# skyhehe123/SA-SSD

Hardware: NVIDIA H100
Metric: KITTI frames/sec (~20k pts, car_cfg voxel grid) (higher is better)
Workload: dtype f32

## Files before the change

### include/sassd_b200.h

```cpp
#ifndef SASSD_B200_H
#define SASSD_B200_H

#include <stddef.h>
#include <stdint.h>

#ifdef __cplusplus
extern "C" {
#endif

typedef void* sassd_stream_t;

enum {
    SASSD_OK = 0,
    SASSD_ERR_ARG = -1,
    SASSD_ERR_LAUNCH = -2,
    SASSD_ERR_WORKSPACE = -3,
    SASSD_ERR_UNSUPPORTED = -4
};

enum {
    SASSD_FLAG_VOXEL_CAP = 1,
    SASSD_FLAG_ROWS_CAP = 2,
    SASSD_FLAG_GUIDED_CAP = 4,
    SASSD_FLAG_NMS_CAP = 8,
// ... 77 lines not shown
                const float* shift, const int32_t* nbr, const int32_t* d_rows, float* out, sassd_stream_t stream);

size_t sassd_gconv_pack_bytes(int taps, int cin, int cout, int precision);
int sassd_gconv_pack(const float* weight, int taps, int cin, int cout, int precision, void* packed,
                     sassd_stream_t stream);

size_t sassd_conv2d_pack_bytes(int taps, int cin, int cout);
int sassd_conv2d_pack(const float* weight, int taps, int cin, int cout, void* packed, sassd_stream_t stream);
typedef struct {
    int32_t batch, H, W;
    int32_t cin, cin_stored;
    int32_t cout, taps, relu;
    int32_t out_f32_stride, out_split_ch;
    int32_t tile_order;
    int32_t n_split;
} sassd_conv2d_desc;
int sassd_conv2d_f16x3(const sassd_conv2d_desc* host_desc, const void* in_split, const void* wpack, const float* scale,
                       const float* shift, float* out_f32, void* out_split, sassd_stream_t stream);
#define SASSD_CONV2D_TILE_H 8
#define SASSD_CONV2D_TILE_W 16
#define SASSD_TILE_DIST_MAX 9
int sassd_conv2d_f16x3_occ(const sassd_conv2d_desc* host_desc, const void* in_split, const void* wpack,
                           const float* scale, const float* shift, float* out_f32, void* out_split,
                           const int32_t* tile_dist, int reach, const float* const_out, int32_t* counters,
                           sassd_stream_t stream);
int sassd_conv2d_f16x3_occ_bg(const sassd_conv2d_desc* host_desc, const void* in_split, const void* wpack,
                              const float* scale, const float* shift, float* out_f32, void* out_split,
                              const int32_t* tile_dist, int reach, const float* const_out, const void* bg_split,
                              const float* bg_f32, int32_t* counters, sassd_stream_t stream);
int sassd_sparse_to_bev_split(const float* feat, const int32_t* coors, const int32_t* d_rows, int rows_cap, int C,
// ... 166 lines not shown
```

### sa-ssd_b200/csrc/conv2d_tma.cu

```cuda
#include <cuda.h>

#include <cstdlib>

#include "tc_common.cuh"

namespace tma {

using namespace tc;

constexpr int TILE_H = SASSD_CONV2D_TILE_H, TILE_W = SASSD_CONV2D_TILE_W;
constexpr int BKC = 64;
constexpr int kConstTile = 1 << 30;
constexpr int kBgTile = 1 << 29;
constexpr int CONS_WARPS = CONS_THREADS / 32;
constexpr int W_LOAD = CONS_WARPS;

constexpr int A_ROWS = TILE_H + 2;
constexpr int A_PLANE_BYTES = A_ROWS * TILE_W * 128;
constexpr int A_STAGE_BYTES = 2 * A_PLANE_BYTES;

constexpr int FRAG_BLOCK_BYTES = 128 * 32;
constexpr int OUT_PITCH = 64 + 4;

template <int BN>
// ... 21 lines not shown
}

struct Conv2dArgs {
    const void* wpack;
    const float* scale;
    const float* shift;
    float* out_f32;
    __half* out_split;
    int batch, H, W, cin, cout, taps, relu, out_f32_stride, out_split_ch;
    const int* tile_dist;
    const float* cvec;
    int reach;
    int* counters;
    int tile_order;
    int nsplit;
};

struct Background {
    const __half* split;
    const float* f32;
};

__device__ __forceinline__ int tile_skip_flag(const Conv2dArgs& p, const Background& bg, int dist, int ty, int tx,
                                              int tiles_y, int tiles_x) {
    if (dist <= p.reach) return 0;
    if (p.reach < 2 || !(ty == 0 || ty == tiles_y - 1 || tx == 0 || tx == tiles_x - 1)) return kConstTile;
    return (bg.split || bg.f32) ? kBgTile : 0;
}

__device__ __forceinline__ void copy_background_unit(const Conv2dArgs& p, const Background& bg, int b, int ty, int tx,
// ... 56 lines not shown
                                                int nthreads) {
    if (!p.out_split || c0 >= p.out_split_ch) return;
    const int vpp = (p.out_split_ch - c0) >> 3;
    const size_t plane = (size_t)p.batch * p.H * p.W * p.out_split_ch;
    const uint4 zero = make_uint4(0u, 0u, 0u, 0u);
    for (int i = tid; i < TILE_H * TILE_W * vpp; i += nthreads) {
        const int pix = i / vpp;
        const int y = ty * TILE_H + pix / TILE_W, x = tx * TILE_W + pix % TILE_W;
        if (y >= p.H || x >= p.W) continue;
        __half* dst = p.out_split + (((size_t)b * p.H + y) * p.W + x) * p.out_split_ch + c0 + 8 * (i % vpp);
        *(uint4*)dst = zero;
        *(uint4*)(dst + plane) = zero;
    }
}

__device__ __forceinline__ void mma_chunk_x3_rs(float (&big)[64], float (&small)[64], const uint32_t (&w)[32],
                                                uint32_t x_hi, uint32_t x_lo) {
    const uint64_t dxh = make_desc(x_hi), dxl = make_desc(x_lo);
#pragma unroll
    for (int k = 0; k < 4; ++k) {
        const uint64_t ko = 2ull * (uint64_t)k;
        const uint32_t wh[4] = {w[8 * k], w[8 * k + 1], w[8 * k + 2], w[8 * k + 3]};
        const uint32_t wl[4] = {w[8 * k + 4], w[8 * k + 5], w[8 * k + 6], w[8 * k + 7]};
        wgmma_rs_n128(small, wh, dxl + ko);
        wgmma_rs_n128(small, wl, dxh + ko);
        wgmma_rs_n128(big, wh, dxh + ko);
    }
}

template <int BN>
__global__ void __launch_bounds__(Cfg2<BN>::THREADS, 1)
conv2d_tma_kernel(const __grid_constant__ CUtensorMap amap, const Conv2dArgs p, const Background bg) {
    using C = Cfg2<BN>;
    constexpr int A_STAGES = C::A_STAGES;
    extern __shared__ uint8_t smem_raw[];
    __shared__ int s_ncomp;
    __shared__ int s_walk[6];
    const uint32_t base = (smem_u32(smem_raw) + 1023u) & ~1023u;
    uint8_t* base_ptr = smem_raw + (base - smem_u32(smem_raw));
    const uint32_t b_ring = base + A_STAGES * A_STAGE_BYTES;
    const uint32_t bar_base = base + C::RING_BYTES;
    auto a_full = [&](int s) { return bar_base + 8u * s; };
    auto a_empty = [&](int s) { return bar_base + 8u * (A_STAGES + s); };
    auto b_full = [&](int s) { return bar_base + 8u * (2 * A_STAGES + s); };
    auto b_empty = [&](int s) { return bar_base + 8u * (2 * A_STAGES + C::B_STAGES + s); };

    pdl_launch_dependents();
    const int warp = __shfl_sync(0xffffffffu, (int)(threadIdx.x >> 5), 0), lane = threadIdx.x & 31;
    const int tiles_x = (p.W + TILE_W - 1) / TILE_W, tiles_y = (p.H + TILE_H - 1) / TILE_H;
    const int ntiles = p.batch * tiles_y * tiles_x;
    const int nsplit = p.nsplit, nunits = ntiles * nsplit;
    const int kchunks = (p.cin + BKC - 1) / BKC;
    const int nchunks = p.taps * kchunks;
    const int ncols = p.taps == 9 ? 3 : 1, nrows = ncols, halo = ncols / 2;

    if (threadIdx.x == 0) {
        for (int s = 0; s < A_STAGES; ++s) { mbar_init(a_full(s), 1); mbar_init(a_empty(s), 2); }
        for (int s = 0; s < C::B_STAGES; ++s) { mbar_init(b_full(s), 1); mbar_init(b_empty(s), 2); }
        fence_barrier_init();
        asm volatile("prefetch.tensormap [%0];" ::"l"(&amap) : "memory");
        s_walk[0] = s_walk[1] = nunits;
        s_walk[2] = s_walk[4] = nunits + blockIdx.x;
        s_walk[3] = 1;
        s_walk[5] = blockIdx.x;
    }
    __syncthreads();
    pdl_wait();

    uint32_t* verdict = (uint32_t*)(base_ptr + C::RING_BYTES + 256);
    uint16_t* order = (uint16_t*)(verdict + 2 * (C::ORDER_CAP / 32));
    const bool small_map = p.tile_dist != nullptr && ntiles <= C::ORDER_CAP;
    const bool use_order = p.tile_order && small_map;
    if (small_map) {
        const int nslots = (ntiles + 31) / 32;
#pragma unroll 1
        for (int i0 = 4 * warp; i0 < nslots; i0 += 4 * (C::THREADS / 32)) {
            int dist[4];
#pragma unroll
            for (int e = 0; e < 4; ++e) {
// ... 25 lines not shown
                    for (int i = 0; i < nslots; ++i) {
                        const int t = i * 32 + lane;
                        const uint32_t cst = verdict[i], bgm = verdict[C::ORDER_CAP / 32 + i];
                        const bool skip = ((cst | bgm) >> lane) & 1u;
                        const bool take = t < ntiles && (skip == (pass == 1));
                        const uint32_t m = __ballot_sync(0xffffffffu, take);
                        if (take) order[n + __popc(m & ((1u << lane) - 1u))] = word(t, cst, bgm);
                        n += __popc(m);
                    }
                    if (pass == 0 && lane == 0) s_ncomp = n;
                }
                if (lane == 0) {
                    constexpr int kTailAbsorb = 8;
                    const int G = gridDim.x, c = blockIdx.x;
                    const int ucomp = s_ncomp * nsplit;
                    const int heavy = ucomp % G, light = G - heavy;
                    const int absorb = heavy ? min(nunits - ucomp, kTailAbsorb * light) : 0;
                    const int s2 = ucomp + c - heavy, s3 = ucomp + absorb + c;
                    const int first_tail = (c >= heavy && s2 < ucomp + absorb) ? s2 : s3;
                    s_walk[0] = ucomp;
                    s_walk[1] = ucomp + absorb;
                    s_walk[2] = first_tail;
                    s_walk[3] = light;
                    s_walk[4] = s3;
                    s_walk[5] = c < ucomp ? c : first_tail;
                }
            } else {
#pragma unroll 1
                for (int i = 0; i < nslots; ++i) {
                    const int t = i * 32 + lane;
                    if (t < ntiles) order[t] = word(t, verdict[i], verdict[C::ORDER_CAP / 32 + i]);
                }
            }
        }
        __syncthreads();
    }
    auto next_unit = [&](int k) -> int {
        if (k < s_walk[0]) { k += gridDim.x; return k < s_walk[0] ? k : s_walk[2]; }
        if (k < s_walk[1]) { k += s_walk[3]; return k < s_walk[1] ? k : s_walk[4]; }
        return k + gridDim.x;
    };
    auto tile_ref = [&](int k) -> int {
        if (small_map) { const int v = order[k]; return (v & 0x3fff) | ((v & 0xc000) << 15); }
        if (!p.tile_dist) return k;
        return k | tile_skip_flag(p, bg, __ldg(&p.tile_dist[k]), (k / tiles_x) % tiles_y, k % tiles_x, tiles_y, tiles_x);
    };

    if (warp >= W_LOAD) {
        if constexpr (C::RS) {
            setmaxnreg_dec<40>();
            if (warp == W_LOAD + 1 && lane == 0) {
                constexpr uint32_t kStep = 2 * FRAG_BLOCK_BYTES;
                int b_stage = 0;
                uint32_t b_phase = 0;
                for (int k = s_walk[5]; k < nunits; k = next_unit(k)) {
                    if (tile_ref(k / nsplit) & (kConstTile | kBgTile)) continue;
                    const uint8_t* src = (const uint8_t*)p.wpack + (size_t)(k % nsplit) * kStep;
                    for (int q = 0; q < nchunks; ++q) {
                        mbar_wait(b_empty(b_stage), b_phase ^ 1u);
                        mbar_expect_tx(b_full(b_stage), C::B_STAGE_BYTES);
                        const uint32_t dst = b_ring + b_stage * C::B_STAGE_BYTES;
#pragma unroll 1
                        for (int s = 0; s < 4; ++s, src += (size_t)nsplit * kStep)
                            bulk_g2s(dst + s * kStep, src, kStep, b_full(b_stage));
                        if (++b_stage == C::B_STAGES) { b_stage = 0; b_phase ^= 1u; }
                    }
                }
            }
            if (warp != W_LOAD) return;
        }
        if (lane == 0) {
            int a_stage = 0, b_stage = 0;
            uint32_t a_phase = 0, b_phase = 0;
            const uint32_t a_bytes = 2u * (TILE_H + 2 * halo) * TILE_W * 128;
            for (int k = s_walk[5]; k < nunits; k = next_unit(k)) {
                const int ref = tile_ref(k / nsplit), half = k % nsplit;
                if (ref & (kConstTile | kBgTile)) continue;
                const int tile = ref;
                const int b = tile / (tiles_y * tiles_x);
                const int ty = (tile / tiles_x) % tiles_y, tx = tile % tiles_x;
                const int y0 = ty * TILE_H, x0 = tx * TILE_W;
                for (int col = 0; col < ncols; ++col) {
                    const int dx = col - halo;
                    for (int kc = 0; kc < kchunks; ++kc) {
                        mbar_wait(a_empty(a_stage), a_phase ^ 1u);
                        const uint32_t a_hi = base + a_stage * A_STAGE_BYTES;
                        mbar_expect_tx(a_full(a_stage), a_bytes);
                        tma_load_4d(a_hi, &amap, kc * BKC, x0 + dx, y0 - halo, b, a_full(a_stage));
                        tma_load_4d(a_hi + A_PLANE_BYTES, &amap, kc * BKC, x0 + dx, y0 - halo, p.batch + b, a_full(a_stage));
                        if (++a_stage == A_STAGES) { a_stage = 0; a_phase ^= 1u; }
// ... 10 lines not shown
#pragma unroll 1
                                for (int part = 0; part < 2; ++part)
#pragma unroll 1
                                    for (uint32_t o = 0; o < (uint32_t)C::B_TILE_BYTES; o += kPiece)
                                        bulk_g2s(b_dst + part * C::B_TILE_BYTES + o,
                                                 src + (size_t)part * nsplit * C::B_TILE_BYTES + o, kPiece, b_full(b_stage));
                                if (++b_stage == C::B_STAGES) { b_stage = 0; b_phase ^= 1u; }
                            }
                        }
                    }
                }
            }
        }
        if (p.out_split && nsplit * BN < p.out_split_ch) {
            __syncwarp();
            for (int k = s_walk[5]; k < nunits; k = next_unit(k)) {
                if (k % nsplit != nsplit - 1) continue;
                const int tile = tile_ref(k / nsplit) & ~(kConstTile | kBgTile);
                zero_split_tail(p, tile / (tiles_y * tiles_x), (tile / tiles_x) % tiles_y, tile % tiles_x, nsplit * BN,
                                lane, 32);
            }
        }
    } else {
        if constexpr (C::RS) setmaxnreg_inc<232>();
        const int wg = threadIdx.x >> 7, t = threadIdx.x & 127;
        const int rl0 = wg * 64 + (t >> 5) * 16 + ((t & 31) >> 2);
        const size_t plane = (size_t)p.batch * p.H * p.W * p.out_split_ch;
        float big[BN / 2], small[BN / 2];
        int a_stage = 0, b_stage = 0;
        uint32_t a_phase = 0, b_phase = 0;
        int computed = 0;
        for (int k = s_walk[5]; k < nunits; k = next_unit(k)) {
            const int ref = tile_ref(k / nsplit), n_off = (k % nsplit) * BN;
            const int tile = ref & ~(kConstTile | kBgTile);
            const bool const_tile = (ref & kConstTile) != 0;
            const int b = tile / (tiles_y * tiles_x);
            const int ty = (tile / tiles_x) % tiles_y, tx = tile % tiles_x;
            if (ref & kBgTile) continue;
            if (const_tile) {
                const int ncols = min(BN, p.out_split_ch - n_off);
                if (p.out_split && !p.out_f32 && (ncols == 64 || ncols == 128 || ncols == 256)) {
                    store_constant_unit<CONS_WARPS>(p, b, ty, tx, n_off, ncols, warp, lane);
                    continue;
                }
            } else {
                if (k % nsplit == 0) ++computed;
#pragma unroll
                for (int i = 0; i < BN / 2; ++i) { big[i] = 0.f; small[i] = 0.f; }
                int prev_b = -1, prev_a = -1, row = 0;
                if constexpr (C::RS) {
                    auto load_w = [&](uint32_t (&w)[32]) {
                        mbar_wait(b_full(b_stage), b_phase);
                        const uint32_t sw = (t & 4) * 4u;
                        const uint32_t src = b_ring + b_stage * C::B_STAGE_BYTES + wg * FRAG_BLOCK_BYTES + t * 32;
#pragma unroll
                        for (int s = 0; s < 4; ++s) {
                            const uint4 x = lds_v4(src + s * 2 * FRAG_BLOCK_BYTES + sw);
                            const uint4 y = lds_v4(src + s * 2 * FRAG_BLOCK_BYTES + (sw ^ 16u));
                            const uint4 h = sw ? y : x, l = sw ? x : y;
                            w[8 * s] = h.x; w[8 * s + 1] = h.y; w[8 * s + 2] = h.z; w[8 * s + 3] = h.w;
                            w[8 * s + 4] = l.x; w[8 * s + 5] = l.y; w[8 * s + 6] = l.z; w[8 * s + 7] = l.w;
                        }
                        named_bar_sync(3 + wg, 128);
                        if (t == 0) mbar_arrive(b_empty(b_stage));
                        if (++b_stage == C::B_STAGES) { b_stage = 0; b_phase ^= 1u; }
                    };
                    auto chunk = [&](uint32_t (&w)[32], uint32_t (&w_next)[32], int ch) {
                        if (row == 0) mbar_wait(a_full(a_stage), a_phase);
                        const uint32_t xh = base + a_stage * A_STAGE_BYTES + (uint32_t)row * (TILE_W * 128u);
                        wgmma_fence();
                        mma_chunk_x3_rs(big, small, w, xh, xh + A_PLANE_BYTES);
                        wgmma_commit();
                        wgmma_wait<1>();
                        fence_regs<32>(w_next);
                        if (t == 0 && prev_a >= 0) mbar_arrive(a_empty(prev_a));
                        if (ch + 1 < nchunks) load_w(w_next);
                        prev_a = -1;
                        if (++row == nrows) {
                            row = 0;
                            prev_a = a_stage;
                            if (++a_stage == A_STAGES) { a_stage = 0; a_phase ^= 1u; }
                        }
                    };
                    uint32_t wa[32], wb[32];
                    load_w(wa);
                    for (int ch = 0; ch < nchunks; ch += 2) {
                        chunk(wa, wb, ch);
// ... 24 lines not shown
                            row = 0;
                            prev_a = a_stage;
                            if (++a_stage == A_STAGES) { a_stage = 0; a_phase ^= 1u; }
                        }
                    }
                }
                wgmma_wait<0>();
                fence_regs<BN / 2>(big);
                fence_regs<BN / 2>(small);
                if (t == 0) {
                    if (prev_b >= 0) mbar_arrive(b_empty(prev_b));
                    if (prev_a >= 0) mbar_arrive(a_empty(prev_a));
                }
            }
            if constexpr (C::RS) {
                float* stage = (float*)(base_ptr + A_STAGES * A_STAGE_BYTES + C::B_STAGES * C::B_STAGE_BYTES) +
                               wg * (TILE_H * TILE_W * OUT_PITCH);
                const int m0 = 16 * (t >> 5) + ((t & 31) >> 2), c_wg = n_off + 64 * wg;
                float cv[2], sc[2], sh[2];
#pragma unroll
                for (int i = 0; i < 2; ++i) {
                    const int n = c_wg + m0 + 8 * i;
                    cv[i] = const_tile && n < p.cout ? __ldg(&p.cvec[n]) : 0.f;
                    sc[i] = p.scale && n < p.cout ? __ldg(&p.scale[n]) : 1.f;
                    sh[i] = p.shift && n < p.cout ? __ldg(&p.shift[n]) : 0.f;
                }
                named_bar_sync(1 + wg, 128);
#pragma unroll
                for (int j = 0; j < 16; ++j)
#pragma unroll
                    for (int i = 0; i < 2; ++i)
#pragma unroll
                        for (int e = 0; e < 2; ++e) {
                            float o = cv[i];
                            if (!const_tile) {
                                o = fmaf(__fadd_rn(big[4 * j + 2 * i + e], small[4 * j + 2 * i + e] * (1.f / kF16LoScale)),
                                         sc[i], sh[i]);
                                if (p.relu) o = fmaxf(o, 0.f);
                                if (c_wg + m0 + 8 * i >= p.cout) o = 0.f;
                            }
                            stage[(8 * j + 2 * (t & 3) + e) * OUT_PITCH + m0 + 8 * i] = o;
                        }
                named_bar_sync(1 + wg, 128);
                if (p.out_f32) {
                    for (int v = t; v < TILE_H * TILE_W * 16; v += 128) {
                        const int pix = v >> 4, c = 4 * (v & 15), n = c_wg + c;
                        const int y = ty * TILE_H + pix / TILE_W, x = tx * TILE_W + pix % TILE_W;
                        if (n >= p.out_f32_stride || y >= p.H || x >= p.W) continue;
                        *(float4*)(p.out_f32 + (((size_t)b * p.H + y) * p.W + x) * p.out_f32_stride + n) =
                            *(const float4*)(stage + pix * OUT_PITCH + c);
                    }
                }
                if (p.out_split) {
                    for (int v = t; v < TILE_H * TILE_W * 8; v += 128) {
                        const int pix = v >> 3, c = 8 * (v & 7), n = c_wg + c;
                        const int y = ty * TILE_H + pix / TILE_W, x = tx * TILE_W + pix % TILE_W;
                        if (n >= p.out_split_ch || y >= p.H || x >= p.W) continue;
                        const float4 f0 = *(const float4*)(stage + pix * OUT_PITCH + c);
                        const float4 f1 = *(const float4*)(stage + pix * OUT_PITCH + c + 4);
                        uint4 hi, lo;
                        split_f16x2(f0.x, f0.y, hi.x, lo.x);
                        split_f16x2(f0.z, f0.w, hi.y, lo.y);
                        split_f16x2(f1.x, f1.y, hi.z, lo.z);
                        split_f16x2(f1.z, f1.w, hi.w, lo.w);
                        __half* dst = p.out_split + (((size_t)b * p.H + y) * p.W + x) * p.out_split_ch + n;
                        *(uint4*)dst = hi;
                        *(uint4*)(dst + plane) = lo;
                    }
                }
            } else {
#pragma unroll
// ... 25 lines not shown
                        const size_t pix = ((size_t)b * p.H + y) * p.W + x;
                        if (p.out_f32 && n < p.out_f32_stride)
                            *(float2*)(p.out_f32 + pix * p.out_f32_stride + n) = make_float2(o0, o1);
                        if (p.out_split && n < p.out_split_ch) {
                            uint32_t h, l;
                            split_f16x2(o0, o1, h, l);
                            __half* dst = p.out_split + pix * p.out_split_ch + n;
                            *(uint32_t*)dst = h;
                            *(uint32_t*)(dst + plane) = l;
                        }
                    }
                }
            }
        }
        if (bg.split || bg.f32) {
            for (int k = s_walk[5]; k < nunits; k = next_unit(k)) {
                const int ref = tile_ref(k / nsplit);
                if (!(ref & kBgTile)) continue;
                const int tile = ref & ~kBgTile;
                copy_background_unit(p, bg, tile / (tiles_y * tiles_x), (tile / tiles_x) % tiles_y, tile % tiles_x,
                                     (k % nsplit) * BN, BN, threadIdx.x, CONS_THREADS);
            }
        }
        if (p.counters && threadIdx.x == 0) {
            if (computed) atomicAdd(&p.counters[0], computed);
            if (blockIdx.x == 0) atomicAdd(&p.counters[1], ntiles);
        }
    }
}

typedef CUresult (*EncodeTiledFn)(CUtensorMap*, CUtensorMapDataType, cuuint32_t, void*, const cuuint64_t*,
// ... 115 lines not shown
    cuuint64_t strides[3] = {(cuuint64_t)d->cin_stored * 2, (cuuint64_t)d->W * d->cin_stored * 2,
                             (cuuint64_t)d->H * d->W * d->cin_stored * 2};
    cuuint32_t box[4] = {(cuuint32_t)BKC, (cuuint32_t)TILE_W, (cuuint32_t)(d->taps == 9 ? A_ROWS : TILE_H), 1u};
    cuuint32_t estr[4] = {1u, 1u, 1u, 1u};
    CUresult rc = enc(&map, CU_TENSOR_MAP_DATA_TYPE_FLOAT16, 4, const_cast<void*>(in_split), dims, strides, box, estr,
                      CU_TENSOR_MAP_INTERLEAVE_NONE, CU_TENSOR_MAP_SWIZZLE_128B, CU_TENSOR_MAP_L2_PROMOTION_L2_256B,
                      CU_TENSOR_MAP_FLOAT_OOB_FILL_NONE);
    if (rc != CUDA_SUCCESS) return SASSD_ERR_LAUNCH;
    Conv2dArgs a;
    a.wpack = wpack; a.scale = scale; a.shift = shift; a.out_f32 = out_f32; a.out_split = (__half*)out_split;
    a.batch = d->batch; a.H = d->H; a.W = d->W; a.cin = d->cin; a.cout = d->cout; a.taps = d->taps; a.relu = d->relu;
    a.out_f32_stride = d->out_f32_stride; a.out_split_ch = d->out_split_ch;
    a.tile_dist = tile_dist; a.reach = reach; a.cvec = const_out; a.counters = counters;
    a.tile_order = d->tile_order;
    a.nsplit = 1;
    const Background bg = {out_split ? (const __half*)bg_split : nullptr, out_f32 ? bg_f32 : nullptr};
    cudaStream_t stream = (cudaStream_t)stream_;
    if (d->cout <= 32) return launch2<32>(map, a, bg, stream);
    if (d->cout <= 64) return launch2<64>(map, a, bg, stream);
    if (d->cout <= 128) return launch2<128>(map, a, bg, stream);
    a.nsplit = 2;
    return launch2<128>(map, a, bg, stream);
}

__global__ void sparse_to_bev_split_kernel(const float4* __restrict__ feat, const int4* __restrict__ coors,
                                           const int* __restrict__ d_rows, int rows_cap, int C4, int D, int H, int W,
                                           size_t plane, __half* __restrict__ bev, int* __restrict__ tile_dist) {
    const int rows = min(*d_rows, rows_cap);
    const long long total = (long long)rows * C4;
    for (long long i = blockIdx.x * (long long)blockDim.x + threadIdx.x; i < total;
// ... 25 lines not shown
```

### sa-ssd_b200/csrc/tc_common.cuh

```cuda
#pragma once
#include <cuda_fp16.h>

#include "common.cuh"

#include <cstdlib>
#include <utility>

namespace tc {

constexpr int BM = 128;
constexpr int BK = 32;
constexpr int A_TILE_BYTES = BM * 128;
constexpr int CONS_THREADS = 256;

__device__ __forceinline__ uint32_t smem_u32(const void* p) { return (uint32_t)__cvta_generic_to_shared(p); }

__device__ __forceinline__ void mbar_init(uint32_t bar, uint32_t count) {
    asm volatile("mbarrier.init.shared::cta.b64 [%0], %1;" ::"r"(bar), "r"(count));
}
__device__ __forceinline__ void mbar_arrive(uint32_t bar) {
    asm volatile("mbarrier.arrive.shared::cta.b64 _, [%0];" ::"r"(bar) : "memory");
}
__device__ __forceinline__ void mbar_expect_tx(uint32_t bar, uint32_t bytes) {
    asm volatile("mbarrier.arrive.expect_tx.shared::cta.b64 _, [%0], %1;" ::"r"(bar), "r"(bytes) : "memory");
// ... 99 lines not shown
    asm volatile(
        "{\n\t.reg .pred p;\n\tsetp.ne.b32 p, %34, 0;\n\t"
        "wgmma.mma_async.sync.aligned.m64n64k8.f32.tf32.tf32 {%0, %1, %2, %3, %4, %5, %6, %7, %8, %9, %10, %11, %12, %13, %14, %15, %16, %17, %18, %19, %20, %21, %22, %23, %24, %25, %26, %27, %28, %29, %30, %31}, %32, %33, p, 1, 1;\n\t}\n"
        : "+f"(d[0]), "+f"(d[1]), "+f"(d[2]), "+f"(d[3]), "+f"(d[4]), "+f"(d[5]), "+f"(d[6]), "+f"(d[7]), "+f"(d[8]), "+f"(d[9]), "+f"(d[10]), "+f"(d[11]), "+f"(d[12]), "+f"(d[13]), "+f"(d[14]), "+f"(d[15]), "+f"(d[16]), "+f"(d[17]), "+f"(d[18]), "+f"(d[19]), "+f"(d[20]), "+f"(d[21]), "+f"(d[22]), "+f"(d[23]), "+f"(d[24]), "+f"(d[25]), "+f"(d[26]), "+f"(d[27]), "+f"(d[28]), "+f"(d[29]), "+f"(d[30]), "+f"(d[31])
        : "l"(da), "l"(db), "r"(scale_d) : "memory");
}
template <>
__device__ __forceinline__ void wgmma<0, 128>(float (&d)[64], uint64_t da, uint64_t db, uint32_t scale_d) {
    asm volatile(
        "{\n\t.reg .pred p;\n\tsetp.ne.b32 p, %66, 0;\n\t"
        "wgmma.mma_async.sync.aligned.m64n128k8.f32.tf32.tf32 {%0, %1, %2, %3, %4, %5, %6, %7, %8, %9, %10, %11, %12, %13, %14, %15, %16, %17, %18, %19, %20, %21, %22, %23, %24, %25, %26, %27, %28, %29, %30, %31, %32, %33, %34, %35, %36, %37, %38, %39, %40, %41, %42, %43, %44, %45, %46, %47, %48, %49, %50, %51, %52, %53, %54, %55, %56, %57, %58, %59, %60, %61, %62, %63}, %64, %65, p, 1, 1;\n\t}\n"
        : "+f"(d[0]), "+f"(d[1]), "+f"(d[2]), "+f"(d[3]), "+f"(d[4]), "+f"(d[5]), "+f"(d[6]), "+f"(d[7]), "+f"(d[8]), "+f"(d[9]), "+f"(d[10]), "+f"(d[11]), "+f"(d[12]), "+f"(d[13]), "+f"(d[14]), "+f"(d[15]), "+f"(d[16]), "+f"(d[17]), "+f"(d[18]), "+f"(d[19]), "+f"(d[20]), "+f"(d[21]), "+f"(d[22]), "+f"(d[23]), "+f"(d[24]), "+f"(d[25]), "+f"(d[26]), "+f"(d[27]), "+f"(d[28]), "+f"(d[29]), "+f"(d[30]), "+f"(d[31]), "+f"(d[32]), "+f"(d[33]), "+f"(d[34]), "+f"(d[35]), "+f"(d[36]), "+f"(d[37]), "+f"(d[38]), "+f"(d[39]), "+f"(d[40]), "+f"(d[41]), "+f"(d[42]), "+f"(d[43]), "+f"(d[44]), "+f"(d[45]), "+f"(d[46]), "+f"(d[47]), "+f"(d[48]), "+f"(d[49]), "+f"(d[50]), "+f"(d[51]), "+f"(d[52]), "+f"(d[53]), "+f"(d[54]), "+f"(d[55]), "+f"(d[56]), "+f"(d[57]), "+f"(d[58]), "+f"(d[59]), "+f"(d[60]), "+f"(d[61]), "+f"(d[62]), "+f"(d[63])
        : "l"(da), "l"(db), "r"(scale_d) : "memory");
}

__device__ __forceinline__ void wgmma_rs_n128(float (&d)[64], const uint32_t (&a)[4], uint64_t db) {
    asm volatile(
        "{\n\t.reg .pred p;\n\tsetp.ne.b32 p, 1, 0;\n\t"
        "wgmma.mma_async.sync.aligned.m64n128k16.f32.f16.f16 {%0, %1, %2, %3, %4, %5, %6, %7, %8, %9, %10, %11, %12, %13, %14, %15, %16, %17, %18, %19, %20, %21, %22, %23, %24, %25, %26, %27, %28, %29, %30, %31, %32, %33, %34, %35, %36, %37, %38, %39, %40, %41, %42, %43, %44, %45, %46, %47, %48, %49, %50, %51, %52, %53, %54, %55, %56, %57, %58, %59, %60, %61, %62, %63}, {%64, %65, %66, %67}, %68, p, 1, 1, 0;\n\t}\n"
        : "+f"(d[0]), "+f"(d[1]), "+f"(d[2]), "+f"(d[3]), "+f"(d[4]), "+f"(d[5]), "+f"(d[6]), "+f"(d[7]), "+f"(d[8]), "+f"(d[9]), "+f"(d[10]), "+f"(d[11]), "+f"(d[12]), "+f"(d[13]), "+f"(d[14]), "+f"(d[15]), "+f"(d[16]), "+f"(d[17]), "+f"(d[18]), "+f"(d[19]), "+f"(d[20]), "+f"(d[21]), "+f"(d[22]), "+f"(d[23]), "+f"(d[24]), "+f"(d[25]), "+f"(d[26]), "+f"(d[27]), "+f"(d[28]), "+f"(d[29]), "+f"(d[30]), "+f"(d[31]), "+f"(d[32]), "+f"(d[33]), "+f"(d[34]), "+f"(d[35]), "+f"(d[36]), "+f"(d[37]), "+f"(d[38]), "+f"(d[39]), "+f"(d[40]), "+f"(d[41]), "+f"(d[42]), "+f"(d[43]), "+f"(d[44]), "+f"(d[45]), "+f"(d[46]), "+f"(d[47]), "+f"(d[48]), "+f"(d[49]), "+f"(d[50]), "+f"(d[51]), "+f"(d[52]), "+f"(d[53]), "+f"(d[54]), "+f"(d[55]), "+f"(d[56]), "+f"(d[57]), "+f"(d[58]), "+f"(d[59]), "+f"(d[60]), "+f"(d[61]), "+f"(d[62]), "+f"(d[63])
        : "r"(a[0]), "r"(a[1]), "r"(a[2]), "r"(a[3]), "l"(db) : "memory");
}
template <int R>
__device__ __forceinline__ void fence_regs(uint32_t (&r)[R]) {
#pragma unroll
    for (int i = 0; i < R; ++i) asm volatile("" : "+r"(r[i])::"memory");
}
template <int N>
__device__ __forceinline__ void setmaxnreg_dec() { asm volatile("setmaxnreg.dec.sync.aligned.u32 %0;" ::"n"(N)); }
template <int N>
__device__ __forceinline__ void setmaxnreg_inc() { asm volatile("setmaxnreg.inc.sync.aligned.u32 %0;" ::"n"(N)); }
__device__ __forceinline__ void named_bar_sync(int id, int nthreads) {
    asm volatile("bar.sync %0, %1;" ::"r"(id), "r"(nthreads) : "memory");
}
__device__ __forceinline__ uint4 lds_v4(uint32_t addr) {
    uint4 v;
// ... 77 lines not shown
```

### sa-ssd_b200/lib.py

```python
import ctypes
import os

from . import build as _build

c_int, c_float, c_size_t, c_void_p = ctypes.c_int, ctypes.c_float, ctypes.c_size_t, ctypes.c_void_p


class VoxelParams(ctypes.Structure):
    _fields_ = [("voxel_size", c_float * 3), ("range_min", c_float * 3), ("grid", ctypes.c_int32 * 3),
                ("max_points", ctypes.c_int32), ("max_voxels", ctypes.c_int32)]


class Conv2dDesc(ctypes.Structure):
    _fields_ = [(n, ctypes.c_int32) for n in ("batch", "H", "W", "cin", "cin_stored", "cout", "taps", "relu",
                                              "out_f32_stride", "out_split_ch", "tile_order", "n_split")]


class SpconvDesc(ctypes.Structure):
    _fields_ = [(n, ctypes.c_int32) for n in ("cin", "cout", "taps", "rows_cap", "in_rows_cap", "relu", "out_ch",
                                              "out_f32_stride")]


class GConvDesc(ctypes.Structure):
    _fields_ = [(n, ctypes.c_int32) for n in ("mode", "precision", "cin", "cout", "taps", "in_stride", "out_stride",
                                              "rows_cap", "batch", "H", "W", "relu")]


class KittiEvalDesc(ctypes.Structure):
    _fields_ = ([(n, ctypes.c_int32) for n in ("nsets", "nframes", "nclass", "ndiff", "nover", "max_nd", "max_ng")]
                + [(n, c_void_p) for n in ("gt_off", "dt_off", "ov_off", "gt_dc", "gt_bbox", "dt_bbox", "dt_score",
# ... 152 lines not shown
```

### sa-ssd_b200/ops.py

```python
import collections
import ctypes
import os
import math

import numpy as np
import torch

from . import lib as _lib
from .lib import Conv2dDesc, SpconvDesc
from .lib import (GCONV_CONV2D, GCONV_ROWS, GCONV_TABLE, PREC_F16X3, PREC_FP32, PREC_TF32X3, GConvDesc, VoxelParams,
                  check)

NMS_CAP = 4096
DEFAULT_PRECISION = PREC_F16X3


def _L():
    return _lib.load()


def _stream():
    return ctypes.c_void_p(torch.cuda.current_stream().cuda_stream)


# ... 629 lines not shown
        return (self.planes[0].float() + self.planes[1].float() * (1.0 / 2048.0))[..., : self.channels].contiguous()

    @staticmethod
    def from_float(x):
        B, H, W, C = x.shape
        cs = (C + 63) // 64 * 64
        hi = x.half()
        lo = ((x - hi.float()) * 2048.0).half()
        planes = torch.zeros((2, B, H, W, cs), dtype=torch.float16, device=x.device)
        planes[0, ..., :C] = hi
        planes[1, ..., :C] = lo
        return SplitMap(planes, C)


TILE_OCCUPANCY = os.environ.get("SASSD_TMA_OCC", "1") != "0"
CONV2D_TILE_ORDER = 0
CONV2D_COUNTERS = None
_TILE_FAR = 1 << 20


def _tile_dist(batch, H, W, device):
    if not TILE_OCCUPANCY:
        return None
    th, tw = _lib.CONV2D_TILE_H, _lib.CONV2D_TILE_W
    return torch.full((batch * ((H + th - 1) // th) * ((W + tw - 1) // tw),), _TILE_FAR, dtype=torch.int32, device=device)


def tile_skipping_valid(H, W, reach):
    th, tw = _lib.CONV2D_TILE_H, _lib.CONV2D_TILE_W
    if reach > _lib.TILE_DIST_MAX:
# ... 61 lines not shown
    dist = _tile_dist(batch, H, W, feat.device)
    _call("sassd_sparse_to_bev_split", None, _ptr(feat), _ptr(coors), _ptr(d_rows), feat.shape[0], C, D, H, W, batch,
          _ptr(planes), _ptr(dist), _stream())
    return SplitMap(planes, D * C, dist)


def conv2d_split(x, weight, scale, shift, relu, cout, out_split=True, out_f32=False):
    B, H, W, cin = x.shape
    taps = weight.shape[0]
    wp = conv2d_pack_cached(weight)
    d = Conv2dDesc()
    d.batch, d.H, d.W, d.cin, d.cin_stored = B, H, W, cin, x.planes.shape[-1]
    d.cout, d.taps, d.relu = cout, taps, 1 if relu else 0
    d.tile_order = CONV2D_TILE_ORDER
    d.n_split = 0
    osp = of = None
    if out_split:
        cs = (cout + 63) // 64 * 64
        osp = torch.empty((2, B, H, W, cs), dtype=torch.float16, device=x.device)
        d.out_split_ch = cs
    if out_f32:
        stride = (cout + 3) // 4 * 4
        of = torch.empty((B, H, W, stride), dtype=torch.float32, device=x.device)
        d.out_f32_stride = stride
    label = "conv2d_tma[taps=%d %d->%d]" % (taps, cin, cout)
    dist = x.tile_dist if TILE_OCCUPANCY else None
    reach, cvec, bg_sp, bg_f = 0, None, None, None
    if dist is not None:
        reach = x.reach + (1 if taps == 9 else 0)
        if not tile_skipping_valid(H, W, reach):
# ... 59 lines not shown
```

Measured before the change: 905.9.

## Split tail work units into half-tile units to balance the persistent conv2d schedule

Adds an optional half-unit mode to the persistent TMA conv2d kernel. When the number of computed units leaves an odd final wave, R units are each split into two 64-pixel halves. Each half runs m64n64 wgmma instructions on a row-offset slice of the A tile and writes only its half of the output. The aim is to shorten the last wave's tail imbalance across CTAs, at the cost of more complex index mapping and a branch inside the fused inline-asm chunk, which now also folds the fence and commit in.

```diff
diff --git a/include/sassd_b200.h b/include/sassd_b200.h
--- a/include/sassd_b200.h
+++ b/include/sassd_b200.h
@@ -115,6 +115,7 @@
     int32_t out_f32_stride, out_split_ch;
     int32_t tile_order;
     int32_t n_split;
+    int32_t whole_units;
 } sassd_conv2d_desc;
 int sassd_conv2d_f16x3(const sassd_conv2d_desc* host_desc, const void* in_split, const void* wpack, const float* scale,
                        const float* shift, float* out_f32, void* out_split, sassd_stream_t stream);
diff --git a/sa-ssd_b200/csrc/conv2d_tma.cu b/sa-ssd_b200/csrc/conv2d_tma.cu
--- a/sa-ssd_b200/csrc/conv2d_tma.cu
+++ b/sa-ssd_b200/csrc/conv2d_tma.cu
@@ -59,6 +59,7 @@
     int* counters;
     int tile_order;
     int nsplit;
+    int half_units;
 };
 
 struct Background {
@@ -145,20 +146,6 @@
     }
 }
 
-__device__ __forceinline__ void mma_chunk_x3_rs(float (&big)[64], float (&small)[64], const uint32_t (&w)[32],
-                                                uint32_t x_hi, uint32_t x_lo) {
-    const uint64_t dxh = make_desc(x_hi), dxl = make_desc(x_lo);
-#pragma unroll
-    for (int k = 0; k < 4; ++k) {
-        const uint64_t ko = 2ull * (uint64_t)k;
-        const uint32_t wh[4] = {w[8 * k], w[8 * k + 1], w[8 * k + 2], w[8 * k + 3]};
-        const uint32_t wl[4] = {w[8 * k + 4], w[8 * k + 5], w[8 * k + 6], w[8 * k + 7]};
-        wgmma_rs_n128(small, wh, dxl + ko);
-        wgmma_rs_n128(small, wl, dxh + ko);
-        wgmma_rs_n128(big, wh, dxh + ko);
-    }
-}
-
 template <int BN>
 __global__ void __launch_bounds__(Cfg2<BN>::THREADS, 1)
 conv2d_tma_kernel(const __grid_constant__ CUtensorMap amap, const Conv2dArgs p, const Background bg) {
@@ -166,7 +153,7 @@
     constexpr int A_STAGES = C::A_STAGES;
     extern __shared__ uint8_t smem_raw[];
     __shared__ int s_ncomp;
-    __shared__ int s_walk[6];
+    __shared__ int s_walk[8];
     const uint32_t base = (smem_u32(smem_raw) + 1023u) & ~1023u;
     uint8_t* base_ptr = smem_raw + (base - smem_u32(smem_raw));
     const uint32_t b_ring = base + A_STAGES * A_STAGE_BYTES;
@@ -194,6 +181,8 @@
         s_walk[2] = s_walk[4] = nunits + blockIdx.x;
         s_walk[3] = 1;
         s_walk[5] = blockIdx.x;
+        s_walk[6] = nunits;
+        s_walk[7] = 0;
     }
     __syncthreads();
     pdl_wait();
@@ -249,16 +238,21 @@
                     constexpr int kTailAbsorb = 8;
                     const int G = gridDim.x, c = blockIdx.x;
                     const int ucomp = s_ncomp * nsplit;
-                    const int heavy = ucomp % G, light = G - heavy;
+                    const int T = (2 * ucomp + G - 1) / G, R_odd = ucomp - (T / 2) * G;
+                    const int R = (C::RS && p.half_units && p.taps == 9 && (T & 1) && 3 * R_odd <= G) ? R_odd : 0;
+                    const int vcomp = ucomp + R;
+                    const int heavy = vcomp % G, light = G - heavy;
                     const int absorb = heavy ? min(nunits - ucomp, kTailAbsorb * light) : 0;
-                    const int s2 = ucomp + c - heavy, s3 = ucomp + absorb + c;
-                    const int first_tail = (c >= heavy && s2 < ucomp + absorb) ? s2 : s3;
-                    s_walk[0] = ucomp;
-                    s_walk[1] = ucomp + absorb;
+                    const int s2 = vcomp + c - heavy, s3 = vcomp + absorb + c;
+                    const int first_tail = (c >= heavy && s2 < vcomp + absorb) ? s2 : s3;
+                    s_walk[0] = vcomp;
+                    s_walk[1] = vcomp + absorb;
                     s_walk[2] = first_tail;
                     s_walk[3] = light;
                     s_walk[4] = s3;
-                    s_walk[5] = c < ucomp ? c : first_tail;
+                    s_walk[5] = c < vcomp ? c : first_tail;
+                    s_walk[6] = ucomp - R;
+                    s_walk[7] = R;
                 }
             } else {
 #pragma unroll 1
@@ -270,10 +264,18 @@
         }
         __syncthreads();
     }
+    const int npos = nunits + s_walk[7];
     auto next_unit = [&](int k) -> int {
         if (k < s_walk[0]) { k += gridDim.x; return k < s_walk[0] ? k : s_walk[2]; }
         if (k < s_walk[1]) { k += s_walk[3]; return k < s_walk[1] ? k : s_walk[4]; }
         return k + gridDim.x;
+    };
+    auto unit_of = [&](int k, int& h) -> int {
+        const int d = k - s_walk[6];
+        h = -1;
+        if (d < 0) return k;
+        if (d < 2 * s_walk[7]) { h = d & 1; return s_walk[6] + (d >> 1); }
+        return k - s_walk[7];
     };
     auto tile_ref = [&](int k) -> int {
         if (small_map) { const int v = order[k]; return (v & 0x3fff) | ((v & 0xc000) << 15); }
@@ -288,7 +290,9 @@
                 constexpr uint32_t kStep = 2 * FRAG_BLOCK_BYTES;
                 int b_stage = 0;
                 uint32_t b_phase = 0;
-                for (int k = s_walk[5]; k < nunits; k = next_unit(k)) {
+                for (int pos = s_walk[5]; pos < npos; pos = next_unit(pos)) {
+                    int h;
+                    const int k = unit_of(pos, h);
                     if (tile_ref(k / nsplit) & (kConstTile | kBgTile)) continue;
                     const uint8_t* src = (const uint8_t*)p.wpack + (size_t)(k % nsplit) * kStep;
                     for (int q = 0; q < nchunks; ++q) {
@@ -308,7 +312,9 @@
             int a_stage = 0, b_stage = 0;
             uint32_t a_phase = 0, b_phase = 0;
             const uint32_t a_bytes = 2u * (TILE_H + 2 * halo) * TILE_W * 128;
-            for (int k = s_walk[5]; k < nunits; k = next_unit(k)) {
+            for (int pos = s_walk[5]; pos < npos; pos = next_unit(pos)) {
+                int h;
+                const int k = unit_of(pos, h);
                 const int ref = tile_ref(k / nsplit), half = k % nsplit;
                 if (ref & (kConstTile | kBgTile)) continue;
                 const int tile = ref;
@@ -349,8 +355,10 @@
         }
         if (p.out_split && nsplit * BN < p.out_split_ch) {
             __syncwarp();
-            for (int k = s_walk[5]; k < nunits; k = next_unit(k)) {
-                if (k % nsplit != nsplit - 1) continue;
+            for (int pos = s_walk[5]; pos < npos; pos = next_unit(pos)) {
+                int h;
+                const int k = unit_of(pos, h);
+                if (k % nsplit != nsplit - 1 || h > 0) continue;
                 const int tile = tile_ref(k / nsplit) & ~(kConstTile | kBgTile);
                 zero_split_tail(p, tile / (tiles_y * tiles_x), (tile / tiles_x) % tiles_y, tile % tiles_x, nsplit * BN,
                                 lane, 32);
@@ -365,7 +373,9 @@
         int a_stage = 0, b_stage = 0;
         uint32_t a_phase = 0, b_phase = 0;
         int computed = 0;
-        for (int k = s_walk[5]; k < nunits; k = next_unit(k)) {
+        for (int pos = s_walk[5]; pos < npos; pos = next_unit(pos)) {
+            int h;
+            const int k = unit_of(pos, h);
             const int ref = tile_ref(k / nsplit), n_off = (k % nsplit) * BN;
             const int tile = ref & ~(kConstTile | kBgTile);
             const bool const_tile = (ref & kConstTile) != 0;
@@ -379,7 +389,7 @@
                     continue;
                 }
             } else {
-                if (k % nsplit == 0) ++computed;
+                if (k % nsplit == 0 && h <= 0) ++computed;
 #pragma unroll
                 for (int i = 0; i < BN / 2; ++i) { big[i] = 0.f; small[i] = 0.f; }
                 int prev_b = -1, prev_a = -1, row = 0;
@@ -402,10 +412,8 @@
                     };
                     auto chunk = [&](uint32_t (&w)[32], uint32_t (&w_next)[32], int ch) {
                         if (row == 0) mbar_wait(a_full(a_stage), a_phase);
-                        const uint32_t xh = base + a_stage * A_STAGE_BYTES + (uint32_t)row * (TILE_W * 128u);
-                        wgmma_fence();
-                        mma_chunk_x3_rs(big, small, w, xh, xh + A_PLANE_BYTES);
-                        wgmma_commit();
+                        const uint32_t xh = base + a_stage * A_STAGE_BYTES + (uint32_t)(row + 4 * max(h, 0)) * (TILE_W * 128u);
+                        wgmma_chunk_x3_rs(big, small, w, make_desc(xh), make_desc(xh + A_PLANE_BYTES), h >= 0);
                         wgmma_wait<1>();
                         fence_regs<32>(w_next);
                         if (t == 0 && prev_a >= 0) mbar_arrive(a_empty(prev_a));
@@ -460,6 +468,7 @@
                 }
             }
             if constexpr (C::RS) {
+                const int px0 = h > 0 ? 64 : 0, npix = h >= 0 ? 64 : TILE_H * TILE_W;
                 float* stage = (float*)(base_ptr + A_STAGES * A_STAGE_BYTES + C::B_STAGES * C::B_STAGE_BYTES) +
                                wg * (TILE_H * TILE_W * OUT_PITCH);
                 const int m0 = 16 * (t >> 5) + ((t & 31) >> 2), c_wg = n_off + 64 * wg;
@@ -473,7 +482,8 @@
                 }
                 named_bar_sync(1 + wg, 128);
 #pragma unroll
-                for (int j = 0; j < 16; ++j)
+                for (int j = 0; j < 16; ++j) {
+                    if (8 * j >= npix) break;
 #pragma unroll
                     for (int i = 0; i < 2; ++i)
 #pragma unroll
@@ -487,20 +497,21 @@
                             }
                             stage[(8 * j + 2 * (t & 3) + e) * OUT_PITCH + m0 + 8 * i] = o;
                         }
+                }
                 named_bar_sync(1 + wg, 128);
                 if (p.out_f32) {
-                    for (int v = t; v < TILE_H * TILE_W * 16; v += 128) {
+                    for (int v = t; v < npix * 16; v += 128) {
                         const int pix = v >> 4, c = 4 * (v & 15), n = c_wg + c;
-                        const int y = ty * TILE_H + pix / TILE_W, x = tx * TILE_W + pix % TILE_W;
+                        const int y = ty * TILE_H + (px0 + pix) / TILE_W, x = tx * TILE_W + pix % TILE_W;
                         if (n >= p.out_f32_stride || y >= p.H || x >= p.W) continue;
                         *(float4*)(p.out_f32 + (((size_t)b * p.H + y) * p.W + x) * p.out_f32_stride + n) =
                             *(const float4*)(stage + pix * OUT_PITCH + c);
                     }
                 }
                 if (p.out_split) {
-                    for (int v = t; v < TILE_H * TILE_W * 8; v += 128) {
+                    for (int v = t; v < npix * 8; v += 128) {
                         const int pix = v >> 3, c = 8 * (v & 7), n = c_wg + c;
-                        const int y = ty * TILE_H + pix / TILE_W, x = tx * TILE_W + pix % TILE_W;
+                        const int y = ty * TILE_H + (px0 + pix) / TILE_W, x = tx * TILE_W + pix % TILE_W;
                         if (n >= p.out_split_ch || y >= p.H || x >= p.W) continue;
                         const float4 f0 = *(const float4*)(stage + pix * OUT_PITCH + c);
                         const float4 f1 = *(const float4*)(stage + pix * OUT_PITCH + c + 4);
@@ -556,7 +567,9 @@
             }
         }
         if (bg.split || bg.f32) {
-            for (int k = s_walk[5]; k < nunits; k = next_unit(k)) {
+            for (int pos = s_walk[5]; pos < npos; pos = next_unit(pos)) {
+                int h;
+                const int k = unit_of(pos, h);
                 const int ref = tile_ref(k / nsplit);
                 if (!(ref & kBgTile)) continue;
                 const int tile = ref & ~kBgTile;
@@ -702,6 +715,7 @@
     a.tile_dist = tile_dist; a.reach = reach; a.cvec = const_out; a.counters = counters;
     a.tile_order = d->tile_order;
     a.nsplit = 1;
+    a.half_units = !d->whole_units;
     const Background bg = {out_split ? (const __half*)bg_split : nullptr, out_f32 ? bg_f32 : nullptr};
     cudaStream_t stream = (cudaStream_t)stream_;
     if (d->cout <= 32) return launch2<32>(map, a, bg, stream);
diff --git a/sa-ssd_b200/csrc/tc_common.cuh b/sa-ssd_b200/csrc/tc_common.cuh
--- a/sa-ssd_b200/csrc/tc_common.cuh
+++ b/sa-ssd_b200/csrc/tc_common.cuh
@@ -137,12 +137,45 @@
         : "l"(da), "l"(db), "r"(scale_d) : "memory");
 }
 
-__device__ __forceinline__ void wgmma_rs_n128(float (&d)[64], const uint32_t (&a)[4], uint64_t db) {
-    asm volatile(
-        "{\n\t.reg .pred p;\n\tsetp.ne.b32 p, 1, 0;\n\t"
-        "wgmma.mma_async.sync.aligned.m64n128k16.f32.f16.f16 {%0, %1, %2, %3, %4, %5, %6, %7, %8, %9, %10, %11, %12, %13, %14, %15, %16, %17, %18, %19, %20, %21, %22, %23, %24, %25, %26, %27, %28, %29, %30, %31, %32, %33, %34, %35, %36, %37, %38, %39, %40, %41, %42, %43, %44, %45, %46, %47, %48, %49, %50, %51, %52, %53, %54, %55, %56, %57, %58, %59, %60, %61, %62, %63}, {%64, %65, %66, %67}, %68, p, 1, 1, 0;\n\t}\n"
-        : "+f"(d[0]), "+f"(d[1]), "+f"(d[2]), "+f"(d[3]), "+f"(d[4]), "+f"(d[5]), "+f"(d[6]), "+f"(d[7]), "+f"(d[8]), "+f"(d[9]), "+f"(d[10]), "+f"(d[11]), "+f"(d[12]), "+f"(d[13]), "+f"(d[14]), "+f"(d[15]), "+f"(d[16]), "+f"(d[17]), "+f"(d[18]), "+f"(d[19]), "+f"(d[20]), "+f"(d[21]), "+f"(d[22]), "+f"(d[23]), "+f"(d[24]), "+f"(d[25]), "+f"(d[26]), "+f"(d[27]), "+f"(d[28]), "+f"(d[29]), "+f"(d[30]), "+f"(d[31]), "+f"(d[32]), "+f"(d[33]), "+f"(d[34]), "+f"(d[35]), "+f"(d[36]), "+f"(d[37]), "+f"(d[38]), "+f"(d[39]), "+f"(d[40]), "+f"(d[41]), "+f"(d[42]), "+f"(d[43]), "+f"(d[44]), "+f"(d[45]), "+f"(d[46]), "+f"(d[47]), "+f"(d[48]), "+f"(d[49]), "+f"(d[50]), "+f"(d[51]), "+f"(d[52]), "+f"(d[53]), "+f"(d[54]), "+f"(d[55]), "+f"(d[56]), "+f"(d[57]), "+f"(d[58]), "+f"(d[59]), "+f"(d[60]), "+f"(d[61]), "+f"(d[62]), "+f"(d[63])
-        : "r"(a[0]), "r"(a[1]), "r"(a[2]), "r"(a[3]), "l"(db) : "memory");
+__device__ __forceinline__ void wgmma_chunk_x3_rs(float (&big)[64], float (&small)[64], const uint32_t (&w)[32],
+                                                  uint64_t dxh, uint64_t dxl, uint32_t n64) {
+    asm volatile(
+        "{\n\t.reg .pred p, h;\n\tsetp.ne.b32 p, 1, 0;\n\tsetp.ne.b32 h, %168, 0;\n\t"
+        "@h bra.uni RS_N64;\n\t"
+        "wgmma.fence.sync.aligned;\n\t"
+        "wgmma.mma_async.sync.aligned.m64n128k16.f32.f16.f16 {%64, %65, %66, %67, %68, %69, %70, %71, %72, %73, %74, %75, %76, %77, %78, %79, %80, %81, %82, %83, %84, %85, %86, %87, %88, %89, %90, %91, %92, %93, %94, %95, %96, %97, %98, %99, %100, %101, %102, %103, %104, %105, %106, %107, %108, %109, %110, %111, %112, %113, %114, %115, %116, %117, %118, %119, %120, %121, %122, %123, %124, %125, %126, %127}, {%128, %129, %130, %131}, %164, p, 1, 1, 0;\n\t"
+        "wgmma.mma_async.sync.aligned.m64n128k16.f32.f16.f16 {%64, %65, %66, %67, %68, %69, %70, %71, %72, %73, %74, %75, %76, %77, %78, %79, %80, %81, %82, %83, %84, %85, %86, %87, %88, %89, %90, %91, %92, %93, %94, %95, %96, %97, %98, %99, %100, %101, %102, %103, %104, %105, %106, %107, %108, %109, %110, %111, %112, %113, %114, %115, %116, %117, %118, %119, %120, %121, %122, %123, %124, %125, %126, %127}, {%132, %133, %134, %135}, %160, p, 1, 1, 0;\n\t"
+        "wgmma.mma_async.sync.aligned.m64n128k16.f32.f16.f16 {%0, %1, %2, %3, %4, %5, %6, %7, %8, %9, %10, %11, %12, %13, %14, %15, %16, %17, %18, %19, %20, %21, %22, %23, %24, %25, %26, %27, %28, %29, %30, %31, %32, %33, %34, %35, %36, %37, %38, %39, %40, %41, %42, %43, %44, %45, %46, %47, %48, %49, %50, %51, %52, %53, %54, %55, %56, %57, %58, %59, %60, %61, %62, %63}, {%128, %129, %130, %131}, %160, p, 1, 1, 0;\n\t"
+        "wgmma.mma_async.sync.aligned.m64n128k16.f32.f16.f16 {%64, %65, %66, %67, %68, %69, %70, %71, %72, %73, %74, %75, %76, %77, %78, %79, %80, %81, %82, %83, %84, %85, %86, %87, %88, %89, %90, %91, %92, %93, %94, %95, %96, %97, %98, %99, %100, %101, %102, %103, %104, %105, %106, %107, %108, %109, %110, %111, %112, %113, %114, %115, %116, %117, %118, %119, %120, %121, %122, %123, %124, %125, %126, %127}, {%136, %137, %138, %139}, %165, p, 1, 1, 0;\n\t"
+        "wgmma.mma_async.sync.aligned.m64n128k16.f32.f16.f16 {%64, %65, %66, %67, %68, %69, %70, %71, %72, %73, %74, %75, %76, %77, %78, %79, %80, %81, %82, %83, %84, %85, %86, %87, %88, %89, %90, %91, %92, %93, %94, %95, %96, %97, %98, %99, %100, %101, %102, %103, %104, %105, %106, %107, %108, %109, %110, %111, %112, %113, %114, %115, %116, %117, %118, %119, %120, %121, %122, %123, %124, %125, %126, %127}, {%140, %141, %142, %143}, %161, p, 1, 1, 0;\n\t"
+        "wgmma.mma_async.sync.aligned.m64n128k16.f32.f16.f16 {%0, %1, %2, %3, %4, %5, %6, %7, %8, %9, %10, %11, %12, %13, %14, %15, %16, %17, %18, %19, %20, %21, %22, %23, %24, %25, %26, %27, %28, %29, %30, %31, %32, %33, %34, %35, %36, %37, %38, %39, %40, %41, %42, %43, %44, %45, %46, %47, %48, %49, %50, %51, %52, %53, %54, %55, %56, %57, %58, %59, %60, %61, %62, %63}, {%136, %137, %138, %139}, %161, p, 1, 1, 0;\n\t"
+        "wgmma.mma_async.sync.aligned.m64n128k16.f32.f16.f16 {%64, %65, %66, %67, %68, %69, %70, %71, %72, %73, %74, %75, %76, %77, %78, %79, %80, %81, %82, %83, %84, %85, %86, %87, %88, %89, %90, %91, %92, %93, %94, %95, %96, %97, %98, %99, %100, %101, %102, %103, %104, %105, %106, %107, %108, %109, %110, %111, %112, %113, %114, %115, %116, %117, %118, %119, %120, %121, %122, %123, %124, %125, %126, %127}, {%144, %145, %146, %147}, %166, p, 1, 1, 0;\n\t"
+        "wgmma.mma_async.sync.aligned.m64n128k16.f32.f16.f16 {%64, %65, %66, %67, %68, %69, %70, %71, %72, %73, %74, %75, %76, %77, %78, %79, %80, %81, %82, %83, %84, %85, %86, %87, %88, %89, %90, %91, %92, %93, %94, %95, %96, %97, %98, %99, %100, %101, %102, %103, %104, %105, %106, %107, %108, %109, %110, %111, %112, %113, %114, %115, %116, %117, %118, %119, %120, %121, %122, %123, %124, %125, %126, %127}, {%148, %149, %150, %151}, %162, p, 1, 1, 0;\n\t"
+        "wgmma.mma_async.sync.aligned.m64n128k16.f32.f16.f16 {%0, %1, %2, %3, %4, %5, %6, %7, %8, %9, %10, %11, %12, %13, %14, %15, %16, %17, %18, %19, %20, %21, %22, %23, %24, %25, %26, %27, %28, %29, %30, %31, %32, %33, %34, %35, %36, %37, %38, %39, %40, %41, %42, %43, %44, %45, %46, %47, %48, %49, %50, %51, %52, %53, %54, %55, %56, %57, %58, %59, %60, %61, %62, %63}, {%144, %145, %146, %147}, %162, p, 1, 1, 0;\n\t"
+        "wgmma.mma_async.sync.aligned.m64n128k16.f32.f16.f16 {%64, %65, %66, %67, %68, %69, %70, %71, %72, %73, %74, %75, %76, %77, %78, %79, %80, %81, %82, %83, %84, %85, %86, %87, %88, %89, %90, %91, %92, %93, %94, %95, %96, %97, %98, %99, %100, %101, %102, %103, %104, %105, %106, %107, %108, %109, %110, %111, %112, %113, %114, %115, %116, %117, %118, %119, %120, %121, %122, %123, %124, %125, %126, %127}, {%152, %153, %154, %155}, %167, p, 1, 1, 0;\n\t"
+        "wgmma.mma_async.sync.aligned.m64n128k16.f32.f16.f16 {%64, %65, %66, %67, %68, %69, %70, %71, %72, %73, %74, %75, %76, %77, %78, %79, %80, %81, %82, %83, %84, %85, %86, %87, %88, %89, %90, %91, %92, %93, %94, %95, %96, %97, %98, %99, %100, %101, %102, %103, %104, %105, %106, %107, %108, %109, %110, %111, %112, %113, %114, %115, %116, %117, %118, %119, %120, %121, %122, %123, %124, %125, %126, %127}, {%156, %157, %158, %159}, %163, p, 1, 1, 0;\n\t"
+        "wgmma.mma_async.sync.aligned.m64n128k16.f32.f16.f16 {%0, %1, %2, %3, %4, %5, %6, %7, %8, %9, %10, %11, %12, %13, %14, %15, %16, %17, %18, %19, %20, %21, %22, %23, %24, %25, %26, %27, %28, %29, %30, %31, %32, %33, %34, %35, %36, %37, %38, %39, %40, %41, %42, %43, %44, %45, %46, %47, %48, %49, %50, %51, %52, %53, %54, %55, %56, %57, %58, %59, %60, %61, %62, %63}, {%152, %153, %154, %155}, %163, p, 1, 1, 0;\n\t"
+        "wgmma.commit_group.sync.aligned;\n\t"
+        "bra.uni RS_DONE;\n\t"
+        "RS_N64:\n\t"
+        "wgmma.fence.sync.aligned;\n\t"
+        "wgmma.mma_async.sync.aligned.m64n64k16.f32.f16.f16 {%64, %65, %66, %67, %68, %69, %70, %71, %72, %73, %74, %75, %76, %77, %78, %79, %80, %81, %82, %83, %84, %85, %86, %87, %88, %89, %90, %91, %92, %93, %94, %95}, {%128, %129, %130, %131}, %164, p, 1, 1, 0;\n\t"
+        "wgmma.mma_async.sync.aligned.m64n64k16.f32.f16.f16 {%64, %65, %66, %67, %68, %69, %70, %71, %72, %73, %74, %75, %76, %77, %78, %79, %80, %81, %82, %83, %84, %85, %86, %87, %88, %89, %90, %91, %92, %93, %94, %95}, {%132, %133, %134, %135}, %160, p, 1, 1, 0;\n\t"
+        "wgmma.mma_async.sync.aligned.m64n64k16.f32.f16.f16 {%0, %1, %2, %3, %4, %5, %6, %7, %8, %9, %10, %11, %12, %13, %14, %15, %16, %17, %18, %19, %20, %21, %22, %23, %24, %25, %26, %27, %28, %29, %30, %31}, {%128, %129, %130, %131}, %160, p, 1, 1, 0;\n\t"
+        "wgmma.mma_async.sync.aligned.m64n64k16.f32.f16.f16 {%64, %65, %66, %67, %68, %69, %70, %71, %72, %73, %74, %75, %76, %77, %78, %79, %80, %81, %82, %83, %84, %85, %86, %87, %88, %89, %90, %91, %92, %93, %94, %95}, {%136, %137, %138, %139}, %165, p, 1, 1, 0;\n\t"
+        "wgmma.mma_async.sync.aligned.m64n64k16.f32.f16.f16 {%64, %65, %66, %67, %68, %69, %70, %71, %72, %73, %74, %75, %76, %77, %78, %79, %80, %81, %82, %83, %84, %85, %86, %87, %88, %89, %90, %91, %92, %93, %94, %95}, {%140, %141, %142, %143}, %161, p, 1, 1, 0;\n\t"
+        "wgmma.mma_async.sync.aligned.m64n64k16.f32.f16.f16 {%0, %1, %2, %3, %4, %5, %6, %7, %8, %9, %10, %11, %12, %13, %14, %15, %16, %17, %18, %19, %20, %21, %22, %23, %24, %25, %26, %27, %28, %29, %30, %31}, {%136, %137, %138, %139}, %161, p, 1, 1, 0;\n\t"
+        "wgmma.mma_async.sync.aligned.m64n64k16.f32.f16.f16 {%64, %65, %66, %67, %68, %69, %70, %71, %72, %73, %74, %75, %76, %77, %78, %79, %80, %81, %82, %83, %84, %85, %86, %87, %88, %89, %90, %91, %92, %93, %94, %95}, {%144, %145, %146, %147}, %166, p, 1, 1, 0;\n\t"
+        "wgmma.mma_async.sync.aligned.m64n64k16.f32.f16.f16 {%64, %65, %66, %67, %68, %69, %70, %71, %72, %73, %74, %75, %76, %77, %78, %79, %80, %81, %82, %83, %84, %85, %86, %87, %88, %89, %90, %91, %92, %93, %94, %95}, {%148, %149, %150, %151}, %162, p, 1, 1, 0;\n\t"
+        "wgmma.mma_async.sync.aligned.m64n64k16.f32.f16.f16 {%0, %1, %2, %3, %4, %5, %6, %7, %8, %9, %10, %11, %12, %13, %14, %15, %16, %17, %18, %19, %20, %21, %22, %23, %24, %25, %26, %27, %28, %29, %30, %31}, {%144, %145, %146, %147}, %162, p, 1, 1, 0;\n\t"
+        "wgmma.mma_async.sync.aligned.m64n64k16.f32.f16.f16 {%64, %65, %66, %67, %68, %69, %70, %71, %72, %73, %74, %75, %76, %77, %78, %79, %80, %81, %82, %83, %84, %85, %86, %87, %88, %89, %90, %91, %92, %93, %94, %95}, {%152, %153, %154, %155}, %167, p, 1, 1, 0;\n\t"
+        "wgmma.mma_async.sync.aligned.m64n64k16.f32.f16.f16 {%64, %65, %66, %67, %68, %69, %70, %71, %72, %73, %74, %75, %76, %77, %78, %79, %80, %81, %82, %83, %84, %85, %86, %87, %88, %89, %90, %91, %92, %93, %94, %95}, {%156, %157, %158, %159}, %163, p, 1, 1, 0;\n\t"
+        "wgmma.mma_async.sync.aligned.m64n64k16.f32.f16.f16 {%0, %1, %2, %3, %4, %5, %6, %7, %8, %9, %10, %11, %12, %13, %14, %15, %16, %17, %18, %19, %20, %21, %22, %23, %24, %25, %26, %27, %28, %29, %30, %31}, {%152, %153, %154, %155}, %163, p, 1, 1, 0;\n\t"
+        "wgmma.commit_group.sync.aligned;\n\t"
+        "RS_DONE:\n\t}\n"
+        : "+f"(big[0]), "+f"(big[1]), "+f"(big[2]), "+f"(big[3]), "+f"(big[4]), "+f"(big[5]), "+f"(big[6]), "+f"(big[7]), "+f"(big[8]), "+f"(big[9]), "+f"(big[10]), "+f"(big[11]), "+f"(big[12]), "+f"(big[13]), "+f"(big[14]), "+f"(big[15]), "+f"(big[16]), "+f"(big[17]), "+f"(big[18]), "+f"(big[19]), "+f"(big[20]), "+f"(big[21]), "+f"(big[22]), "+f"(big[23]), "+f"(big[24]), "+f"(big[25]), "+f"(big[26]), "+f"(big[27]), "+f"(big[28]), "+f"(big[29]), "+f"(big[30]), "+f"(big[31]), "+f"(big[32]), "+f"(big[33]), "+f"(big[34]), "+f"(big[35]), "+f"(big[36]), "+f"(big[37]), "+f"(big[38]), "+f"(big[39]), "+f"(big[40]), "+f"(big[41]), "+f"(big[42]), "+f"(big[43]), "+f"(big[44]), "+f"(big[45]), "+f"(big[46]), "+f"(big[47]), "+f"(big[48]), "+f"(big[49]), "+f"(big[50]), "+f"(big[51]), "+f"(big[52]), "+f"(big[53]), "+f"(big[54]), "+f"(big[55]), "+f"(big[56]), "+f"(big[57]), "+f"(big[58]), "+f"(big[59]), "+f"(big[60]), "+f"(big[61]), "+f"(big[62]), "+f"(big[63]), "+f"(small[0]), "+f"(small[1]), "+f"(small[2]), "+f"(small[3]), "+f"(small[4]), "+f"(small[5]), "+f"(small[6]), "+f"(small[7]), "+f"(small[8]), "+f"(small[9]), "+f"(small[10]), "+f"(small[11]), "+f"(small[12]), "+f"(small[13]), "+f"(small[14]), "+f"(small[15]), "+f"(small[16]), "+f"(small[17]), "+f"(small[18]), "+f"(small[19]), "+f"(small[20]), "+f"(small[21]), "+f"(small[22]), "+f"(small[23]), "+f"(small[24]), "+f"(small[25]), "+f"(small[26]), "+f"(small[27]), "+f"(small[28]), "+f"(small[29]), "+f"(small[30]), "+f"(small[31]), "+f"(small[32]), "+f"(small[33]), "+f"(small[34]), "+f"(small[35]), "+f"(small[36]), "+f"(small[37]), "+f"(small[38]), "+f"(small[39]), "+f"(small[40]), "+f"(small[41]), "+f"(small[42]), "+f"(small[43]), "+f"(small[44]), "+f"(small[45]), "+f"(small[46]), "+f"(small[47]), "+f"(small[48]), "+f"(small[49]), "+f"(small[50]), "+f"(small[51]), "+f"(small[52]), "+f"(small[53]), "+f"(small[54]), "+f"(small[55]), "+f"(small[56]), "+f"(small[57]), "+f"(small[58]), "+f"(small[59]), "+f"(small[60]), "+f"(small[61]), "+f"(small[62]), "+f"(small[63])
+        : "r"(w[0]), "r"(w[1]), "r"(w[2]), "r"(w[3]), "r"(w[4]), "r"(w[5]), "r"(w[6]), "r"(w[7]), "r"(w[8]), "r"(w[9]), "r"(w[10]), "r"(w[11]), "r"(w[12]), "r"(w[13]), "r"(w[14]), "r"(w[15]), "r"(w[16]), "r"(w[17]), "r"(w[18]), "r"(w[19]), "r"(w[20]), "r"(w[21]), "r"(w[22]), "r"(w[23]), "r"(w[24]), "r"(w[25]), "r"(w[26]), "r"(w[27]), "r"(w[28]), "r"(w[29]), "r"(w[30]), "r"(w[31]), "l"(dxh + 0ull), "l"(dxh + 2ull), "l"(dxh + 4ull), "l"(dxh + 6ull), "l"(dxl + 0ull), "l"(dxl + 2ull), "l"(dxl + 4ull), "l"(dxl + 6ull), "r"(n64)
+        : "memory");
 }
 template <int R>
 __device__ __forceinline__ void fence_regs(uint32_t (&r)[R]) {
diff --git a/sa-ssd_b200/lib.py b/sa-ssd_b200/lib.py
--- a/sa-ssd_b200/lib.py
+++ b/sa-ssd_b200/lib.py
@@ -13,7 +13,8 @@
 
 class Conv2dDesc(ctypes.Structure):
     _fields_ = [(n, ctypes.c_int32) for n in ("batch", "H", "W", "cin", "cin_stored", "cout", "taps", "relu",
-                                              "out_f32_stride", "out_split_ch", "tile_order", "n_split")]
+                                              "out_f32_stride", "out_split_ch", "tile_order", "n_split",
+                                              "whole_units")]
 
 
 class SpconvDesc(ctypes.Structure):
diff --git a/sa-ssd_b200/ops.py b/sa-ssd_b200/ops.py
--- a/sa-ssd_b200/ops.py
+++ b/sa-ssd_b200/ops.py
@@ -667,6 +667,7 @@
 
 
 TILE_OCCUPANCY = os.environ.get("SASSD_TMA_OCC", "1") != "0"
+TMA_HALF_UNITS = os.environ.get("SASSD_TMA_HALF", "1") != "0"
 CONV2D_TILE_ORDER = 0
 CONV2D_COUNTERS = None
 _TILE_FAR = 1 << 20
@@ -758,6 +759,7 @@
     d.cout, d.taps, d.relu = cout, taps, 1 if relu else 0
     d.tile_order = CONV2D_TILE_ORDER
     d.n_split = 0
+    d.whole_units = 0 if TMA_HALF_UNITS else 1
     osp = of = None
     if out_split:
         cs = (cout + 63) // 64 * 64
```

Result: no change. 913.7, median of 6 (+0.9%).
